# daviyan5/ninpol

Measured on AMD Instinct MI355X. Metric: Mnodes/s interpolated (GLS, 10M-cell hex mesh) + achieved HBM GB/s vs peak, higher is better.
Workload: dtype f64

## Files before the change

### ninpol_amd/csrc/kernels_gls_hex8mf.hip

```cpp
#include <hip/hip_runtime.h>

#include <cstdio>
#include <cstdlib>

#include "device_grid.hpp"
#include "gls_device_math.hpp"
#include "hex8_desc.hpp"
#include "launch.hpp"

namespace nin {

namespace {

using namespace glsmath;

__device__ __forceinline__ double quad_sum(double v) {
    v += dpp_mov<0xB1>(v);
    v += dpp_mov<0x4E>(v);
    return v;
}
template <int L>
__device__ __forceinline__ double quad_bcast(double v) { return dpp_mov<L * 0x55>(v); }

constexpr int NPW = 16;
constexpr int NR = 8, NC = 13;

template <int K>
struct BackLoop {
    static __device__ __forceinline__ void run(const double (&C)[NR][NC], const double (&rinvq)[3], double (&t)[3],
                                               double (&y)[12], int l) {
        constexpr int Q = K / 4, LAM = K % 4;
        const double yk = quad_bcast<LAM>(t[Q] * rinvq[Q]);
        y[K] = yk;
#pragma unroll
        for (int q = 0; q < Q; ++q) t[q] = fma(-C[q][K], yk, t[q]);
        if (LAM > 0) t[Q] = fma((l < LAM) ? -C[Q][K] : 0.0, yk, t[Q]);
        BackLoop<K - 1>::run(C, rinvq, t, y, l);
    }
};
template <>
struct BackLoop<-1> {
    static __device__ __forceinline__ void run(const double (&)[NR][NC], const double (&)[3], double (&)[3], double (&)[12], int) {}
};

#ifdef NIN_W2_FENCE_COLUMNS
#define NIN_W2_COLUMN_FENCE() __builtin_amdgcn_sched_barrier(0)
#else
#define NIN_W2_COLUMN_FENCE() do { } while (0)
#endif
constexpr int W2_SLOTS = 35;
constexpr int W2_WAVE_DOUBLES = W2_SLOTS * 64 + NPW * 8 + 64;

template <int K>
__device__ __forceinline__ void p2_step_lean(double (&C)[NR][NC], double (&rinvq)[3], int l) {
    constexpr int Q = K / 4, LAM = K % 4;
    const bool is_piv = (l == LAM);
    const double xq = (l > LAM) ? C[Q][K] : 0.0;
    double ss = xq * xq;
#pragma unroll
    for (int r = Q + 1; r < NR; ++r) ss = fma(C[r][K], C[r][K], ss);
    ss = quad_sum(ss);
    const double alpha = quad_bcast<LAM>(C[Q][K]);
    const House h = house_unguarded(alpha, ss);
    rinvq[Q] = is_piv ? h.rinv : rinvq[Q];
    const double vq = is_piv ? h.vp : xq;
#pragma unroll
    for (int j = K + 1; j < NC; ++j) {
        double a = vq * C[Q][j];
#pragma unroll
        for (int r = Q + 1; r < NR; ++r) a = fma(C[r][K], C[r][j], a);
        const double w = -(h.g * quad_sum(a));
        C[Q][j] = fma(w, vq, C[Q][j]);
#pragma unroll
        for (int r = Q + 1; r < NR; ++r) C[r][j] = fma(w, C[r][K], C[r][j]);
    }
}
template <int K, int KEND>
struct P2LeanLoop {
    static __device__ __forceinline__ void run(double (&C)[NR][NC], double (&rinvq)[3], int l) {
        p2_step_lean<K>(C, rinvq, l);
        P2LeanLoop<K + 1, KEND>::run(C, rinvq, l);
    }
};
template <int KEND>
struct P2LeanLoop<KEND, KEND> {
    static __device__ __forceinline__ void run(double (&)[NR][NC], double (&)[3], int) {}
};

template <int R0>
__device__ __forceinline__ void w2_column(const double (&P)[10][3], const double (&g3)[3], const double (&cc)[3], const double (&z)[3],
                                          const double (&b)[3], double &u_out, double (&fill)[7]) {
    double w0, w1, w2;
    if (R0 < 0) {
        w0 = -(g3[0] * P[0][0]);
        w1 = -(g3[1] * (w0 * cc[0]));
        w2 = -(g3[2] * fma(w1, cc[2], w0 * cc[1]));
    } else {
        w0 = -(g3[0] * fma(P[R0 + 2][0], b[2], fma(P[R0 + 1][0], b[1], P[R0][0] * b[0])));
        w1 = -(g3[1] * fma(w0, cc[0], fma(P[R0 + 2][1], b[2], fma(P[R0 + 1][1], b[1], P[R0][1] * b[0]))));
        const double d2 = (R0 >= 2) ? fma(P[R0 + 2][2], b[2], fma(P[R0 + 1][2], b[1], P[R0 < 0 ? 0 : R0][2] * b[0]))
                                    : fma(P[R0 + 2][2], b[2], P[R0 + 1][2] * b[1]);
        w2 = -(g3[2] * fma(w1, cc[2], fma(w0, cc[1], d2)));
    }
    double B[10];
#pragma unroll
    for (int r = 0; r < 10; ++r) {
        const bool own = R0 >= 0 && r >= R0 && r < R0 + 3;
        double v = own ? fma(w0, P[r][0], b[own ? r - R0 : 0]) : (R0 < 0 && r == 0) ? fma(w0, P[0][0], 1.0) : w0 * P[r][0];
        if (r >= 1) v = fma(w1, P[r][1], v);
        if (r >= 2) v = fma(w2, P[r][2], v);
        B[r] = v;
    }
    u_out = fma(z[2], B[2], fma(z[1], B[1], z[0] * B[0]));
#pragma unroll
    for (int r = 0; r < 7; ++r) fill[r] = B[3 + r];
}

__device__ __forceinline__ void w2_dma(const void *gptr, uint32_t *row) {
    __builtin_amdgcn_global_load_lds((const __attribute__((address_space(1))) void *)gptr, (__attribute__((address_space(3))) void *)row, 4, 0, 0);
}
__device__ __forceinline__ void w2_dma_wait() { asm volatile("s_waitcnt vmcnt(0)" ::: "memory"); }
__device__ __forceinline__ void w2_stage_a(const int32_t *nodes, const int32_t *desc, int32_t wg, int32_t count, int nd, int l,
                                           uint32_t *row_p, uint32_t *row_dsc) {
    const int32_t idx = wg * NPW + nd;
    const uint32_t sel = (uint32_t)((idx >= 0 && idx < count) ? idx : count - 1);
    w2_dma(nodes + sel, row_p);
    w2_dma(desc + 4 * (size_t)sel + l, row_dsc);
}
__device__ __forceinline__ void w2_stage_b(const GridView &g, uint32_t p, uint32_t *rows_n) {
    w2_dma(g.esup_ptr + p, rows_n);
    w2_dma(g.fsup_ptr + p, rows_n + 64);
    const uint32_t *xw = reinterpret_cast<const uint32_t *>(g.coords) + 6 * (size_t)p;
#pragma unroll
    for (int k = 0; k < 6; ++k) w2_dma(xw + k, rows_n + 64 * (2 + k));
}
__device__ __forceinline__ void w2_stage_c(const GridView &g, uint32_t eb, uint32_t fb, uint32_t dsc, uint32_t *rows_n) {
    w2_dma(g.esup + eb + (dsc & 7), rows_n + 64 * 8);
    w2_dma(g.esup + eb + ((dsc >> 3) & 7), rows_n + 64 * 9);
#pragma unroll
    for (int i = 0; i < 3; ++i) {
        const uint32_t w = dsc >> (6 + 8 * i);
        w2_dma(g.esup + eb + ((w >> 4) & 7), rows_n + 64 * (10 + i));
        w2_dma(g.fsup + fb + (w & 15), rows_n + 64 * (13 + i));
    }
}

#ifdef NIN_W2_TRACE
__device__ unsigned long long nin_w2_trace[4096 * 4];
#endif
template <bool APPLY>
__global__ __launch_bounds__(256, 2) void nin_gls_hex8w2_kernel(GridView g, const int32_t *__restrict__ nodes,
                                                                const int32_t *__restrict__ desc, int32_t count,
                                                                int add_neumann, double *__restrict__ out,
                                                                double *__restrict__ nws, int32_t *__restrict__ queue,
                                                                const double *__restrict__ u_cells, int32_t n_fields,
                                                                double *__restrict__ values) {
    __shared__ double lds_all[4][W2_WAVE_DOUBLES];
    const int lane = threadIdx.x & 63, wave = threadIdx.x >> 6;
    const int l = lane & 3, nd = lane >> 2;
    double *const L = lds_all[wave] + lane;
    double *const wbuf = lds_all[wave] + W2_SLOTS * 64;
    uint32_t *const row_p = reinterpret_cast<uint32_t *>(lds_all[wave] + W2_SLOTS * 64 + NPW * 8);
    uint32_t *const row_dsc = row_p + 64;
    uint32_t *const rows_n = reinterpret_cast<uint32_t *>(lds_all[wave] + 13 * 64);

    const int32_t n_groups = (count + NPW - 1) / NPW;
    int32_t wg_lo, wg_end;
    int32_t *q;
    if ((gridDim.x & 7) == 0) {
        const int32_t xcd = blockIdx.x & 7, per = (n_groups + 7) / 8;
        wg_lo = xcd * per;
        wg_end = (xcd + 1) * per < n_groups ? (xcd + 1) * per : n_groups;
        q = queue + kGlsQueueLine * xcd;
    } else {
        wg_lo = 0;
        wg_end = n_groups;
        q = queue;
    }
    int32_t ticket = 0;
    if (lane == 0) ticket = atomicAdd(q, 1);
    int32_t wg = wg_lo + __builtin_amdgcn_readfirstlane(ticket);
    if (lane == 0) ticket = atomicAdd(q, 1);
    int32_t wg_next = wg_lo + __builtin_amdgcn_readfirstlane(ticket);
    w2_stage_a(nodes, desc, wg, count, nd, l, row_p, row_dsc);
    w2_dma_wait();
    w2_stage_b(g, row_p[lane], rows_n);
    w2_dma_wait();
    w2_stage_c(g, rows_n[lane], rows_n[64 + lane], row_dsc[lane], rows_n);
#ifdef NIN_MF_STAMPS
#ifndef NIN_MF_STAMP_PASS
#define NIN_MF_STAMP_PASS 8
#endif
    unsigned long long stamps[8];
    int n_stamp = 0, pass_no = 0;
#define NIN_MF_STAMP() do { if (n_stamp < 8) { __builtin_amdgcn_sched_barrier(0); stamps[n_stamp++] = __builtin_amdgcn_s_memtime(); __builtin_amdgcn_s_waitcnt(0xC07F); __builtin_amdgcn_sched_barrier(0); } } while (0)
#else
#define NIN_MF_STAMP() do { } while (0)
#endif
#ifdef NIN_W2_TRACE
    const unsigned long long trace_t0 = __builtin_amdgcn_s_memrealtime();
    unsigned trace_passes = 0;
#endif
    while (wg < wg_end) {
        if (lane == 0) ticket = atomicAdd(q, 1);
#ifdef NIN_W2_TRACE
        ++trace_passes;
#endif
#ifdef NIN_MF_STAMPS
        n_stamp = 0;
#endif
        NIN_MF_STAMP();
        const bool valid = wg * NPW + nd < count;
        w2_dma_wait();
        const uint32_t p = row_p[lane], dsc = row_dsc[lane];
        const uint32_t eb = rows_n[lane], fb = rows_n[64 + lane];
        const bool is_neu = (g.flags[p] & 2) != 0;
        double xv[3];
#pragma unroll
        for (int k = 0; k < 3; ++k) xv[k] = __hiloint2double((int)rows_n[64 * (3 + 2 * k) + lane], (int)rows_n[64 * (2 + 2 * k) + lane]);
        uint32_t id[8];
#pragma unroll
        for (int k = 0; k < 8; ++k) id[k] = rows_n[64 * (8 + k) + lane];
        const uint32_t ce = id[0], co = id[1];

        double P[10][3], de[3], dod[3], nb0[3][3], sav[3][2][3];
        {
            double Ke[9];
#pragma unroll
            for (int k = 0; k < 9; ++k) Ke[k] = g.perm[9 * (size_t)ce + k];
            const double dme = g.diff_mag[ce];
#pragma unroll
            for (int t = 0; t < 3; ++t) {
                de[t] = g.centroids[3 * (size_t)ce + t] - xv[t];
                dod[t] = g.centroids[3 * (size_t)co + t] - xv[t];
                P[0][t] = de[t];
            }
#pragma unroll
            for (int i = 0; i < 3; ++i) {
                const uint32_t w = dsc >> (6 + 8 * i);
                const uint32_t cn = id[2 + i], f = id[5 + i];
                const double N0 = (double)g.face_normal[3 * (size_t)f + 0], N1 = (double)g.face_normal[3 * (size_t)f + 1],
                             N2 = (double)g.face_normal[3 * (size_t)f + 2];
                const double T0 = xv[0] - g.face_center[3 * (size_t)f + 0], T1 = xv[1] - g.face_center[3 * (size_t)f + 1],
                             T2 = xv[2] - g.face_center[3 * (size_t)f + 2];
                const double U0 = N1 * T2 - N2 * T1, U1 = N2 * T0 - N0 * T2, U2 = N0 * T1 - N1 * T0;
                const double dmn = g.diff_mag[cn];
                double eta = 0.0;
                eta = dme > eta ? dme : eta;
                eta = dmn > eta ? dmn : eta;
                const double tj = face_tau_sq(U0 * U0 + U1 * U1 + U2 * U2, eta);
                const bool side_a = ((w >> 7) & 1) != 0;
                const double sg = side_a ? -1.0 : 1.0;
                const double *Kn = g.perm + 9 * (size_t)cn;
#pragma unroll
                for (int t = 0; t < 3; ++t) {
                    P[1 + 3 * i][t] = sg * (Ke[t * 3 + 0] * N0 + Ke[t * 3 + 1] * N1 + Ke[t * 3 + 2] * N2);
                    nb0[i][t] = -sg * (Kn[t * 3 + 0] * N0 + Kn[t * 3 + 1] * N1 + Kn[t * 3 + 2] * N2);
                }
                sav[i][0][0] = sg * T0; sav[i][0][1] = sg * T1; sav[i][0][2] = sg * T2;
                sav[i][1][0] = sg * (tj * U0); sav[i][1][1] = sg * (tj * U1); sav[i][1][2] = sg * (tj * U2);
#pragma unroll
                for (int t = 0; t < 3; ++t) { P[2 + 3 * i][t] = sav[i][0][t]; P[3 + 3 * i][t] = sav[i][1][t]; }
            }
        }
        NIN_MF_STAMP();
        w2_stage_a(nodes, desc, wg_next, count, nd, l, row_p, row_dsc);
        double C[NR][NC];
        double u[9], se, F1[7][2], F2[7][3];
        {
            double g3[3], z[3];
            front_panel(P, de, g3, z);
            pin(z[0]); pin(z[1]); pin(z[2]);
            double cc[3];
            cc[0] = P[1][1] * P[1][0];
            cc[1] = P[2][2] * P[2][0];
            cc[2] = P[2][2] * P[2][1];
#pragma unroll
            for (int r = 2; r < 10; ++r) cc[0] = fma(P[r][1], P[r][0], cc[0]);
#pragma unroll
            for (int r = 3; r < 10; ++r) { cc[1] = fma(P[r][2], P[r][0], cc[1]); cc[2] = fma(P[r][2], P[r][1], cc[2]); }
            {
                const double none[3] = {0.0, 0.0, 0.0};
                double fill[7];
                w2_column<-1>(P, g3, cc, z, none, se, fill);
                pin(se);
#pragma unroll
                for (int r = 0; r < 7; ++r) L[64 * r] = fill[r];
            }
            __builtin_amdgcn_sched_barrier(0);
#pragma unroll
            for (int t = 0; t < 3; ++t) {
                const double b[3] = {nb0[0][t], -sav[0][0][t], -sav[0][1][t]};
                double fill[7];
                w2_column<1>(P, g3, cc, z, b, u[t], fill);
                pin(u[t]);
#pragma unroll
                for (int r = 0; r < 7; ++r) L[64 * (7 + 7 * t + r)] = fill[r];
                NIN_W2_COLUMN_FENCE();
            }
            __builtin_amdgcn_sched_barrier(0);
#pragma unroll
            for (int t = 0; t < 3; ++t) {
                const double b[3] = {nb0[1][t], -sav[1][0][t], -sav[1][1][t]};
                double fill[7];
                w2_column<4>(P, g3, cc, z, b, u[3 + t], fill);
                pin(u[3 + t]);
                if (t == 0) {
#pragma unroll
                    for (int r = 0; r < 7; ++r) L[64 * (28 + r)] = fill[r];
                } else {
#pragma unroll
                    for (int r = 0; r < 7; ++r) F1[r][t - 1] = fill[r];
                }
                NIN_W2_COLUMN_FENCE();
            }
            __builtin_amdgcn_sched_barrier(0);
#pragma unroll
            for (int t = 0; t < 3; ++t) {
                const double b[3] = {nb0[2][t], -sav[2][0][t], -sav[2][1][t]};
                double fill[7];
                w2_column<7>(P, g3, cc, z, b, u[6 + t], fill);
                pin(u[6 + t]);
#pragma unroll
                for (int r = 0; r < 7; ++r) F2[r][t] = fill[r];
                NIN_W2_COLUMN_FENCE();
            }
            __builtin_amdgcn_sched_barrier(0);
        }
        NIN_MF_STAMP();
        {
            const bool lt3 = l < 3, lt2 = l < 2, eq0 = l == 0, ge2 = l >= 2, ge1 = l >= 1, eq3 = l == 3;
#pragma unroll
            for (int t = 0; t < 3; ++t) {
#pragma unroll
                for (int r = 0; r < 7; ++r) {
                    const double f1 = (t == 0) ? L[64 * (28 + r)] : F1[r][t == 0 ? 0 : t - 1];
                    const double f0 = L[64 * (7 + 7 * t + r)];
                    C[r][6 + t] = eq0 ? F2[r][t] : (ge2 ? f1 : 0.0);
                    C[r][9 + t] = ge1 ? F2[r][t] : 0.0;
                    C[r][3 + t] = lt2 ? f1 : (eq3 ? f0 : 0.0);
                    C[r][t] = lt3 ? f0 : 0.0;
                }
            }
#pragma unroll
            for (int r = 0; r < 7; ++r) C[r][12] = L[64 * r];
        }
        __builtin_amdgcn_sched_barrier(0);
#pragma unroll
        for (int j = 0; j < 9; ++j) L[64 * j] = u[j];
        L[64 * 9] = se;
#pragma unroll
        for (int s = 0; s < 4; ++s) {
#pragma unroll
            for (int t = 0; t < 3; ++t) C[7][3 * s + t] = (l == s) ? dod[t] : 0.0;
        }
        C[7][12] = 1.0;
        __builtin_amdgcn_sched_barrier(0);

        double rinvq[3] = {0.0, 0.0, 0.0};
        NIN_MF_STAMP();
        w2_dma_wait();
        w2_stage_b(g, row_p[lane], rows_n);
        __builtin_amdgcn_sched_barrier(0);
        P2LeanLoop<0, 6>::run(C, rinvq, l);
        NIN_MF_STAMP();
        __builtin_amdgcn_sched_barrier(0);
        w2_dma_wait();
        w2_stage_c(g, rows_n[lane], rows_n[64 + lane], row_dsc[lane], rows_n);
        __builtin_amdgcn_sched_barrier(0);
        P2LeanLoop<6, 12>::run(C, rinvq, l);
        NIN_MF_STAMP();
        double y[12], t3[3] = {C[0][12], C[1][12], C[2][12]};
        BackLoop<11>::run(C, rinvq, t3, y, l);
        NIN_MF_STAMP();
        double tail = 0.0;
#pragma unroll
        for (int r = 3; r < NR; ++r) tail = fma(C[r][12], C[r][12], tail);
        const double rr = quad_sum(tail);

        double re = 1.0 - L[64 * 9];
#pragma unroll
        for (int i = 0; i < 3; ++i) {
            const bool low = i < 3 - l;
#pragma unroll
            for (int t = 0; t < 3; ++t) re = fma(L[64 * (3 * i + t)], low ? y[3 * i + t] : y[3 * i + 3 + t], re);
        }
        double dots[4];
#pragma unroll
        for (int s = 0; s < 4; ++s) dots[s] = fma(dod[2], y[3 * s + 2], fma(dod[1], y[3 * s + 1], dod[0] * y[3 * s]));
        const double dsel = (l == 0) ? dots[0] : (l == 1) ? dots[1] : (l == 2) ? dots[2] : dots[3];
        const double ro = 1.0 - dsel;
        const double rri = fast_rcp(rr);
        double we = re * rri, wo = ro * rri;
        const bool ok = rr > 0.0;
        we = (ok && __builtin_isfinite(we)) ? we : 0.0;
        wo = (ok && __builtin_isfinite(wo)) ? wo : 0.0;

        wbuf[nd * 8 + (dsc & 7)] = we;
        wbuf[nd * 8 + ((dsc >> 3) & 7)] = wo;
        wave_lds_sync();
        const double nwv = is_neu ? wbuf[nd * 8 + 7] : 0.0;
        const double addv = add_neumann ? nwv : 0.0;
        const double o0 = wbuf[nd * 8 + 2 * l] + addv, o1 = wbuf[nd * 8 + 2 * l + 1] + addv;
        if (APPLY) {
            const size_t c0 = (size_t)g.esup[eb + 2 * l], c1 = (size_t)g.esup[eb + 2 * l + 1];
            for (int32_t f = 0; f < n_fields; ++f) {
                const double *uf = u_cells + (size_t)f * (size_t)g.n_elems;
                const double yv = quad_sum(fma(o1, uf[c1], o0 * uf[c0]));
                if (valid && l == 0) values[(size_t)f * (size_t)g.n_points + p] = yv;
            }
            if (valid && l == 0) nws[p] = nwv;
        } else if (valid) {
            out[eb + 2 * l] = o0;
            out[eb + 2 * l + 1] = o1;
            if (l == 0) nws[p] = nwv;
        }
        wave_lds_sync();
        NIN_MF_STAMP();
#ifdef NIN_MF_STAMPS
        if (blockIdx.x == 0 && threadIdx.x == 0 && ++pass_no == NIN_MF_STAMP_PASS)
            for (int i = 0; i < 8; ++i) nws[nodes[i]] = (double)(stamps[i] - stamps[0]);
#endif
        wg = wg_next;
        wg_next = wg_lo + __builtin_amdgcn_readfirstlane(ticket);
    }
    w2_dma_wait();
#ifdef NIN_W2_TRACE
    if (lane == 0 && blockIdx.x < 1024) {
        unsigned long long *t = nin_w2_trace + 4 * ((size_t)blockIdx.x * 4 + wave);
        t[0] = trace_t0;
        t[1] = __builtin_amdgcn_s_memrealtime();
        t[2] = __builtin_amdgcn_s_getreg((4 << 0) | (0 << 6) | (31 << 11));
        t[3] = trace_passes;
    }
#endif
}

__global__ void k_hex8_desc(GridView g, const int32_t *__restrict__ nodes, int32_t count, int32_t *__restrict__ desc) {
    const int64_t i = (int64_t)blockIdx.x * blockDim.x + threadIdx.x;
    if (i >= count) return;
    int32_t d[4] = {0, 0, 0, 0};
    (void)hex8_descriptor(g, nodes ? nodes[i] : (int32_t)i, d);
#pragma unroll
    for (int l = 0; l < 4; ++l) desc[4 * i + l] = d[l];
}

}

int launch_hex8_desc(const GridView &g, const int32_t *nodes, int32_t count, int32_t *desc, hipStream_t stream) {
    if (count <= 0) return 0;
    hipLaunchKernelGGL(k_hex8_desc, dim3((unsigned)((count + 255) / 256)), dim3(256), 0, stream, g, nodes, count, desc);
    return hipGetLastError() == hipSuccess ? 0 : -3;
}

int launch_gls_hex8mf(const GridView &g, const int32_t *nodes, const int32_t *desc, int32_t count, int add_neumann,
                      double *out, double *nws, int32_t *queue, hipStream_t stream) {
    if (count <= 0) return 0;
    int64_t blocks = ((int64_t)count + 4 * NPW - 1) / (4 * NPW);
    const char *cap_env = getenv("NIN_W2_BLOCKS");
    const int64_t cap2 = cap_env ? atoll(cap_env) : 512;
    if (blocks > cap2) blocks = cap2;
    if (blocks > 8) blocks &= ~(int64_t)7;
    if (getenv("NIN_DEBUG_OCCUPANCY") != nullptr) {
        int nb = -1;
        (void)hipOccupancyMaxActiveBlocksPerMultiprocessor(&nb, nin_gls_hex8w2_kernel<false>, 256, 0);
        fprintf(stderr, "nin_gls_hex8w2_kernel: %d workgroups per CU, %lld launched\n", nb, (long long)blocks);
    }
    hipLaunchKernelGGL(nin_gls_hex8w2_kernel<false>, dim3((unsigned)blocks), dim3(256), 0, stream, g, nodes, desc, count, add_neumann, out, nws, queue,
                       nullptr, 0, nullptr);
#ifdef NIN_W2_TRACE
    if (getenv("NIN_W2_TRACE_FILE") != nullptr) {
        static int calls = 0;
        if (++calls == 6) {
            (void)hipStreamSynchronize(stream);
            static unsigned long long host[4096 * 4];
            (void)hipMemcpyFromSymbol(host, HIP_SYMBOL(nin_w2_trace), sizeof(host));
            FILE *f = fopen(getenv("NIN_W2_TRACE_FILE"), "w");
            for (int64_t b = 0; b < blocks * 4 && b < 4096; ++b)
                fprintf(f, "%lld %llu %llu %llx %llu\n", (long long)b, host[4 * b], host[4 * b + 1], host[4 * b + 2], host[4 * b + 3]);
            fclose(f);
        }
    }
#endif
    return hipGetLastError() == hipSuccess ? 0 : -3;
}

int launch_gls_hex8mf_apply(const GridView &g, const int32_t *nodes, const int32_t *desc, int32_t count, int add_neumann,
                            const double *u_cells, int32_t n_fields, double *values, double *nws, int32_t *queue, hipStream_t stream) {
    if (count <= 0) return 0;
    int64_t blocks = ((int64_t)count + 4 * NPW - 1) / (4 * NPW);
    if (blocks > 512) blocks = 512;
    if (blocks > 8) blocks &= ~(int64_t)7;
    hipLaunchKernelGGL(nin_gls_hex8w2_kernel<true>, dim3((unsigned)blocks), dim3(256), 0, stream, g, nodes, desc, count, add_neumann,
                       nullptr, nws, queue, u_cells, n_fields, values);
    return hipGetLastError() == hipSuccess ? 0 : -3;
}

const char *kernel_name_gls_hex8mf() { return "nin_gls_hex8w2_kernel<false>"; }

}
```

Before: 2191.

## Deepen gather pipeline: prefetch geometry into registers and share neighbor data via DPP

```diff
diff --git a/ninpol_amd/csrc/kernels_gls_hex8mf.hip b/ninpol_amd/csrc/kernels_gls_hex8mf.hip
--- a/ninpol_amd/csrc/kernels_gls_hex8mf.hip
+++ b/ninpol_amd/csrc/kernels_gls_hex8mf.hip
@@ -119,7 +119,11 @@
 __device__ __forceinline__ void w2_dma(const void *gptr, uint32_t *row) {
     __builtin_amdgcn_global_load_lds((const __attribute__((address_space(1))) void *)gptr, (__attribute__((address_space(3))) void *)row, 4, 0, 0);
 }
-__device__ __forceinline__ void w2_dma_wait() { asm volatile("s_waitcnt vmcnt(0)" ::: "memory"); }
+__device__ __forceinline__ void w2_dma_wait() {
+    __builtin_amdgcn_sched_barrier(0);
+    asm volatile("s_waitcnt vmcnt(0)" ::: "memory");
+    __builtin_amdgcn_sched_barrier(0);
+}
 __device__ __forceinline__ void w2_stage_a(const int32_t *nodes, const int32_t *desc, int32_t wg, int32_t count, int nd, int l,
                                            uint32_t *row_p, uint32_t *row_dsc) {
     const int32_t idx = wg * NPW + nd;
@@ -127,23 +131,52 @@
     w2_dma(nodes + sel, row_p);
     w2_dma(desc + 4 * (size_t)sel + l, row_dsc);
 }
-__device__ __forceinline__ void w2_stage_b(const GridView &g, uint32_t p, uint32_t *rows_n) {
-    w2_dma(g.esup_ptr + p, rows_n);
-    w2_dma(g.fsup_ptr + p, rows_n + 64);
+__device__ __forceinline__ void w2_stage_b(const GridView &g, uint32_t p, uint32_t *rows_b) {
+    w2_dma(g.esup_ptr + p, rows_b);
+    w2_dma(g.fsup_ptr + p, rows_b + 64);
+}
+__device__ __forceinline__ void w2_stage_c(const GridView &g, uint32_t p, uint32_t eb, uint32_t fb, uint32_t dsc, uint32_t *rows_n) {
     const uint32_t *xw = reinterpret_cast<const uint32_t *>(g.coords) + 6 * (size_t)p;
 #pragma unroll
     for (int k = 0; k < 6; ++k) w2_dma(xw + k, rows_n + 64 * (2 + k));
-}
-__device__ __forceinline__ void w2_stage_c(const GridView &g, uint32_t eb, uint32_t fb, uint32_t dsc, uint32_t *rows_n) {
     w2_dma(g.esup + eb + (dsc & 7), rows_n + 64 * 8);
     w2_dma(g.esup + eb + ((dsc >> 3) & 7), rows_n + 64 * 9);
 #pragma unroll
+    for (int i = 0; i < 3; ++i) w2_dma(g.fsup + fb + ((dsc >> (6 + 8 * i)) & 15), rows_n + 64 * (10 + i));
+}
+struct W2Geo {
+    double Ke[9], dme, ce[3];
+    double Ko[9], dmo, co[3];
+    double fc[3][3];
+    float fn[3][3];
+    uint32_t flags;
+};
+__device__ __forceinline__ void w2_stage_d(const GridView &g, const uint32_t *row_p, const uint32_t *rows_n, int lane, W2Geo &q) {
+    q.flags = g.flags[row_p[lane]];
+    const uint32_t ce = rows_n[64 * 8 + lane], co = rows_n[64 * 9 + lane];
+#pragma unroll
+    for (int k = 0; k < 9; ++k) { q.Ke[k] = g.perm[9 * (size_t)ce + k]; q.Ko[k] = g.perm[9 * (size_t)co + k]; }
+    q.dme = g.diff_mag[ce];
+    q.dmo = g.diff_mag[co];
+#pragma unroll
+    for (int t = 0; t < 3; ++t) { q.ce[t] = g.centroids[3 * (size_t)ce + t]; q.co[t] = g.centroids[3 * (size_t)co + t]; }
+#pragma unroll
     for (int i = 0; i < 3; ++i) {
-        const uint32_t w = dsc >> (6 + 8 * i);
-        w2_dma(g.esup + eb + ((w >> 4) & 7), rows_n + 64 * (10 + i));
-        w2_dma(g.fsup + fb + (w & 15), rows_n + 64 * (13 + i));
-    }
-}
+        const uint32_t f = rows_n[64 * (10 + i) + lane];
+#pragma unroll
+        for (int t = 0; t < 3; ++t) { q.fn[i][t] = g.face_normal[3 * (size_t)f + t]; q.fc[i][t] = g.face_center[3 * (size_t)f + t]; }
+    }
+}
+template <int I>
+__device__ __forceinline__ double w2_across(double v) { return dpp_mov<I == 0 ? 0x40 : I == 1 ? 0xA5 : 0xFE>(v); }
+
+#ifndef W2_C_STEP
+#define W2_C_STEP 0
+#endif
+#ifndef W2_D_STEP
+#define W2_D_STEP 6
+#endif
+static_assert(W2_C_STEP >= 0 && W2_C_STEP < W2_D_STEP && W2_D_STEP <= 12, "level 2 before level 3, both in phase 2");
 
 #ifdef NIN_W2_TRACE
 __device__ unsigned long long nin_w2_trace[4096 * 4];
@@ -162,6 +195,7 @@
     double *const wbuf = lds_all[wave] + W2_SLOTS * 64;
     uint32_t *const row_p = reinterpret_cast<uint32_t *>(lds_all[wave] + W2_SLOTS * 64 + NPW * 8);
     uint32_t *const row_dsc = row_p + 64;
+    uint32_t *const rows_b = reinterpret_cast<uint32_t *>(wbuf);
     uint32_t *const rows_n = reinterpret_cast<uint32_t *>(lds_all[wave] + 13 * 64);
 
     const int32_t n_groups = (count + NPW - 1) / NPW;
@@ -182,11 +216,18 @@
     int32_t wg = wg_lo + __builtin_amdgcn_readfirstlane(ticket);
     if (lane == 0) ticket = atomicAdd(q, 1);
     int32_t wg_next = wg_lo + __builtin_amdgcn_readfirstlane(ticket);
+    W2Geo geo;
     w2_stage_a(nodes, desc, wg, count, nd, l, row_p, row_dsc);
     w2_dma_wait();
-    w2_stage_b(g, row_p[lane], rows_n);
+    w2_stage_b(g, row_p[lane], rows_b);
     w2_dma_wait();
-    w2_stage_c(g, rows_n[lane], rows_n[64 + lane], row_dsc[lane], rows_n);
+    {
+        const uint32_t eb0 = rows_b[lane];
+        rows_n[lane] = eb0;
+        w2_stage_c(g, row_p[lane], eb0, rows_b[64 + lane], row_dsc[lane], rows_n);
+    }
+    w2_dma_wait();
+    w2_stage_d(g, row_p, rows_n, lane, geo);
 #ifdef NIN_MF_STAMPS
 #ifndef NIN_MF_STAMP_PASS
 #define NIN_MF_STAMP_PASS 8
@@ -202,7 +243,6 @@
     unsigned trace_passes = 0;
 #endif
     while (wg < wg_end) {
-        if (lane == 0) ticket = atomicAdd(q, 1);
 #ifdef NIN_W2_TRACE
         ++trace_passes;
 #endif
@@ -211,50 +251,51 @@
 #endif
         NIN_MF_STAMP();
         const bool valid = wg * NPW + nd < count;
-        w2_dma_wait();
-        const uint32_t p = row_p[lane], dsc = row_dsc[lane];
-        const uint32_t eb = rows_n[lane], fb = rows_n[64 + lane];
-        const bool is_neu = (g.flags[p] & 2) != 0;
+        __builtin_amdgcn_s_waitcnt(0x0F70);
+#ifdef NIN_MF_STAMP_SPLIT
+        NIN_MF_STAMP();
+#define NIN_MF_STAMP_BACK() do { } while (0)
+#else
+#define NIN_MF_STAMP_BACK() NIN_MF_STAMP()
+#endif
+        const uint32_t p = row_p[lane], dsc = row_dsc[lane], eb = rows_n[lane];
         double xv[3];
 #pragma unroll
         for (int k = 0; k < 3; ++k) xv[k] = __hiloint2double((int)rows_n[64 * (3 + 2 * k) + lane], (int)rows_n[64 * (2 + 2 * k) + lane]);
-        uint32_t id[8];
-#pragma unroll
-        for (int k = 0; k < 8; ++k) id[k] = rows_n[64 * (8 + k) + lane];
-        const uint32_t ce = id[0], co = id[1];
+        const bool is_neu = (geo.flags & 2) != 0;
+        __builtin_amdgcn_s_waitcnt(0xC07F);
+        w2_stage_a(nodes, desc, wg_next, count, nd, l, row_p, row_dsc);
+        __builtin_amdgcn_sched_barrier(0);
 
         double P[10][3], de[3], dod[3], nb0[3][3], sav[3][2][3];
         {
-            double Ke[9];
-#pragma unroll
-            for (int k = 0; k < 9; ++k) Ke[k] = g.perm[9 * (size_t)ce + k];
-            const double dme = g.diff_mag[ce];
+            const double dme = geo.dme;
 #pragma unroll
             for (int t = 0; t < 3; ++t) {
-                de[t] = g.centroids[3 * (size_t)ce + t] - xv[t];
-                dod[t] = g.centroids[3 * (size_t)co + t] - xv[t];
+                de[t] = geo.ce[t] - xv[t];
+                dod[t] = geo.co[t] - xv[t];
                 P[0][t] = de[t];
             }
 #pragma unroll
             for (int i = 0; i < 3; ++i) {
                 const uint32_t w = dsc >> (6 + 8 * i);
-                const uint32_t cn = id[2 + i], f = id[5 + i];
-                const double N0 = (double)g.face_normal[3 * (size_t)f + 0], N1 = (double)g.face_normal[3 * (size_t)f + 1],
-                             N2 = (double)g.face_normal[3 * (size_t)f + 2];
-                const double T0 = xv[0] - g.face_center[3 * (size_t)f + 0], T1 = xv[1] - g.face_center[3 * (size_t)f + 1],
-                             T2 = xv[2] - g.face_center[3 * (size_t)f + 2];
+                const double N0 = (double)geo.fn[i][0], N1 = (double)geo.fn[i][1], N2 = (double)geo.fn[i][2];
+                const double T0 = xv[0] - geo.fc[i][0], T1 = xv[1] - geo.fc[i][1], T2 = xv[2] - geo.fc[i][2];
                 const double U0 = N1 * T2 - N2 * T1, U1 = N2 * T0 - N0 * T2, U2 = N0 * T1 - N1 * T0;
-                const double dmn = g.diff_mag[cn];
+                auto across = [&](double v) { return i == 0 ? w2_across<0>(v) : i == 1 ? w2_across<1>(v) : w2_across<2>(v); };
+                const double dmn = across(geo.dmo);
                 double eta = 0.0;
                 eta = dme > eta ? dme : eta;
                 eta = dmn > eta ? dmn : eta;
                 const double tj = face_tau_sq(U0 * U0 + U1 * U1 + U2 * U2, eta);
                 const bool side_a = ((w >> 7) & 1) != 0;
                 const double sg = side_a ? -1.0 : 1.0;
-                const double *Kn = g.perm + 9 * (size_t)cn;
+                double Kn[9];
+#pragma unroll
+                for (int k = 0; k < 9; ++k) Kn[k] = across(geo.Ko[k]);
 #pragma unroll
                 for (int t = 0; t < 3; ++t) {
-                    P[1 + 3 * i][t] = sg * (Ke[t * 3 + 0] * N0 + Ke[t * 3 + 1] * N1 + Ke[t * 3 + 2] * N2);
+                    P[1 + 3 * i][t] = sg * (geo.Ke[t * 3 + 0] * N0 + geo.Ke[t * 3 + 1] * N1 + geo.Ke[t * 3 + 2] * N2);
                     nb0[i][t] = -sg * (Kn[t * 3 + 0] * N0 + Kn[t * 3 + 1] * N1 + Kn[t * 3 + 2] * N2);
                 }
                 sav[i][0][0] = sg * T0; sav[i][0][1] = sg * T1; sav[i][0][2] = sg * T2;
@@ -263,8 +304,17 @@
                 for (int t = 0; t < 3; ++t) { P[2 + 3 * i][t] = sav[i][0][t]; P[3 + 3 * i][t] = sav[i][1][t]; }
             }
         }
-        NIN_MF_STAMP();
-        w2_stage_a(nodes, desc, wg_next, count, nd, l, row_p, row_dsc);
+#pragma unroll
+        for (int r = 0; r < 10; ++r) { pin(P[r][0]); pin(P[r][1]); pin(P[r][2]); }
+#pragma unroll
+        for (int i = 0; i < 3; ++i) { pin(nb0[i][0]); pin(nb0[i][1]); pin(nb0[i][2]); }
+        NIN_MF_STAMP();
+#ifndef W2_B_LATE
+        w2_dma_wait();
+        w2_stage_b(g, row_p[lane], rows_b);
+#endif
+        if (lane == 0) ticket = atomicAdd(q, 1);
+        __builtin_amdgcn_sched_barrier(0);
         double C[NR][NC];
         double u[9], se, F1[7][2], F2[7][3];
         {
@@ -328,6 +378,10 @@
             __builtin_amdgcn_sched_barrier(0);
         }
         NIN_MF_STAMP();
+#ifdef W2_B_LATE
+        w2_dma_wait();
+        w2_stage_b(g, row_p[lane], rows_b);
+#endif
         {
             const bool lt3 = l < 3, lt2 = l < 2, eq0 = l == 0, ge2 = l >= 2, ge1 = l >= 1, eq3 = l == 3;
 #pragma unroll
@@ -359,20 +413,30 @@
 
         double rinvq[3] = {0.0, 0.0, 0.0};
         NIN_MF_STAMP();
+        __builtin_amdgcn_sched_barrier(0);
+        P2LeanLoop<0, W2_C_STEP>::run(C, rinvq, l);
+        __builtin_amdgcn_sched_barrier(0);
         w2_dma_wait();
-        w2_stage_b(g, row_p[lane], rows_n);
-        __builtin_amdgcn_sched_barrier(0);
-        P2LeanLoop<0, 6>::run(C, rinvq, l);
+        {
+            const uint32_t ebn = rows_b[lane];
+            rows_n[lane] = ebn;
+            w2_stage_c(g, row_p[lane], ebn, rows_b[64 + lane], row_dsc[lane], rows_n);
+        }
+        __builtin_amdgcn_sched_barrier(0);
+        P2LeanLoop<W2_C_STEP, W2_D_STEP>::run(C, rinvq, l);
         NIN_MF_STAMP();
         __builtin_amdgcn_sched_barrier(0);
         w2_dma_wait();
-        w2_stage_c(g, rows_n[lane], rows_n[64 + lane], row_dsc[lane], rows_n);
-        __builtin_amdgcn_sched_barrier(0);
-        P2LeanLoop<6, 12>::run(C, rinvq, l);
+        int32_t wg_after = wg_lo + __builtin_amdgcn_readfirstlane(ticket);
+        asm volatile("" : "+s"(wg_after));
+        __builtin_amdgcn_sched_barrier(0);
+        w2_stage_d(g, row_p, rows_n, lane, geo);
+        __builtin_amdgcn_sched_barrier(0);
+        P2LeanLoop<W2_D_STEP, 12>::run(C, rinvq, l);
         NIN_MF_STAMP();
         double y[12], t3[3] = {C[0][12], C[1][12], C[2][12]};
         BackLoop<11>::run(C, rinvq, t3, y, l);
-        NIN_MF_STAMP();
+        NIN_MF_STAMP_BACK();
         double tail = 0.0;
 #pragma unroll
         for (int r = 3; r < NR; ++r) tail = fma(C[r][12], C[r][12], tail);
@@ -422,7 +486,7 @@
             for (int i = 0; i < 8; ++i) nws[nodes[i]] = (double)(stamps[i] - stamps[0]);
 #endif
         wg = wg_next;
-        wg_next = wg_lo + __builtin_amdgcn_readfirstlane(ticket);
+        wg_next = wg_after;
     }
     w2_dma_wait();
 #ifdef NIN_W2_TRACE
```

After: 2232 (median of 6 runs). 1.9% higher.
